# edouardoyallon/acco

Hardware: NVIDIA H100
Metric: tokens/sec (device-timed, max over ranks) Llama ACCO bf16 sharded-Adam, 8x1024 tokens per GPU per micro-batch (higher is better)
Workload: dtype bf16

## Files before the change

### acco_b200/csrc/attention_wgmma.cu

```cuda
#include <cuda.h>
#include <cuda_bf16.h>
#include <cuda_runtime.h>
#include <math.h>
#include <stdint.h>

#include "wgmma.cuh"

namespace acco_attn {

using namespace acco_tc;

constexpr int HD = 64;
constexpr int LDS = HD + 8;
constexpr float LOG2E = 1.4426950408889634f;
constexpr float LN2 = 0.6931471805599453f;

typedef __nv_bfloat16 bf16;

__device__ __forceinline__ uint32_t pack2(float a, float b) {
    __nv_bfloat162 h = __floats2bfloat162_rn(a, b);
    return *reinterpret_cast<uint32_t*>(&h);
}
__device__ __forceinline__ uint32_t ld32(const bf16* p) { return *reinterpret_cast<const uint32_t*>(p); }

__device__ __forceinline__ void mma16816(float (&c)[4], const uint32_t (&a)[4], uint32_t b0, uint32_t b1) {
    asm volatile("mma.sync.aligned.m16n8k16.row.col.f32.bf16.bf16.f32 {%0,%1,%2,%3}, {%4,%5,%6,%7}, {%8,%9}, {%0,%1,%2,%3};"
                 : "+f"(c[0]), "+f"(c[1]), "+f"(c[2]), "+f"(c[3])
                 : "r"(a[0]), "r"(a[1]), "r"(a[2]), "r"(a[3]), "r"(b0), "r"(b1));
}

template <int NB, int KB>
__device__ __forceinline__ void warp_mma_ss(float (&acc)[NB][4], const bf16* A, const bf16* B, int lane) {
    const int g = lane >> 2, t = lane & 3;
#pragma unroll
    for (int kb = 0; kb < KB; ++kb) {
        uint32_t a[4];
        const bf16* a0 = A + g * LDS + kb * 16 + 2 * t;
        a[0] = ld32(a0); a[1] = ld32(a0 + 8 * LDS); a[2] = ld32(a0 + 8); a[3] = ld32(a0 + 8 * LDS + 8);
#pragma unroll
        for (int nb = 0; nb < NB; ++nb) {
            const bf16* b = B + (nb * 8 + g) * LDS + kb * 16 + 2 * t;
            mma16816(acc[nb], a, ld32(b), ld32(b + 8));
        }
    }
}
template <int NB>
__device__ __forceinline__ void warp_mma_rs(float (&acc)[NB][4], const float (&p)[8][4], const bf16* B, int lane) {
    const int g = lane >> 2, t = lane & 3;
#pragma unroll
    for (int kb = 0; kb < 4; ++kb) {
        uint32_t a[4];
        a[0] = pack2(p[2 * kb][0], p[2 * kb][1]);
        a[1] = pack2(p[2 * kb][2], p[2 * kb][3]);
        a[2] = pack2(p[2 * kb + 1][0], p[2 * kb + 1][1]);
        a[3] = pack2(p[2 * kb + 1][2], p[2 * kb + 1][3]);
#pragma unroll
        for (int nb = 0; nb < NB; ++nb) {
            const bf16* b = B + (nb * 8 + g) * LDS + kb * 16 + 2 * t;
            mma16816(acc[nb], a, ld32(b), ld32(b + 8));
        }
    }
}

__device__ __forceinline__ void load_tile(bf16* dst, const bf16* src, long long ld, int rows, int valid, int tid, int nthr) {
    for (int i = tid; i < rows * 8; i += nthr) {
        const int r = i >> 3, c = (i & 7) * 8;
        uint4 v = make_uint4(0, 0, 0, 0);
        if (r < valid) v = *reinterpret_cast<const uint4*>(src + (long long)r * ld + c);
        *reinterpret_cast<uint4*>(dst + r * LDS + c) = v;
    }
}
__device__ __forceinline__ void load_tile_t(bf16* dst, const bf16* src, long long ld, int rows, int tid, int nthr) {
    for (int i = tid; i < rows * 8; i += nthr) {
        const int r = i >> 3, c = (i & 7) * 8;
        const uint4 v = *reinterpret_cast<const uint4*>(src + (long long)r * ld + c);
        const bf16* e = reinterpret_cast<const bf16*>(&v);
#pragma unroll
        for (int j = 0; j < 8; ++j) dst[(c + j) * LDS + r] = e[j];
    }
}

__device__ __forceinline__ bool visible(int q, int kv, int window) { return kv <= q && kv > q - window; }

struct FwdParams {
    CUtensorMap map_q;
    CUtensorMap map_k;
    CUtensorMap map_v;
    bf16* o;
    long long ld_o;
    float* lse;
    int B, S, Hq, Hk, window;
    float scale;
    const int* seg;
};

constexpr int FWD_Q = 128, FWD_KV = 64, FWD_THREADS = 256;
constexpr int FWD_TILE_KV = FWD_KV * HD * 2;
constexpr int FWD_SMEM = FWD_Q * HD * 2 + 2 * 2 * FWD_TILE_KV + 1024  + 64 ;

__device__ __forceinline__ void wgmma_m64n64k16_rs_tb(float (&d)[32], const uint32_t (&a)[4], uint64_t db) {
    asm volatile(
        "{\n\t.reg .pred p;\n\tsetp.ne.b32 p, %37, 0;\n\twgmma.mma_async.sync.aligned.m64n64k16.f32.bf16.bf16 "
// ... 116 lines not shown
                a[3] = pack2(sc[8 * kk + 6], sc[8 * kk + 7]);
                wgmma_m64n64k16_rs_tb(o, a, make_smem_desc(v_addr + kk * 2048, 8192 >> 4, 1024 >> 4));
            }
            wgmma_commit();
            wgmma_wait<0>();
            reg_fence(o);
        }
        __syncthreads();
        if (tid == 0 && j + 2 <= j_hi) issue(j + 2);
    }
#pragma unroll
    for (int r = 0; r < 2; ++r) {
        const int q = qr[r];
        const float inv = l_run[r] > 0.f ? 1.f / l_run[r] : 0.f;
        bf16* dst = P.o + ((long long)row0 + q) * P.ld_o + h * HD + 2 * t;
#pragma unroll
        for (int nb = 0; nb < 8; ++nb)
            *reinterpret_cast<uint32_t*>(dst + nb * 8) = pack2(o[4 * nb + 2 * r] * inv, o[4 * nb + 2 * r + 1] * inv);
        if (t == 0) P.lse[((long long)b * P.Hq + h) * P.S + q] = (m_run[r] + log2f(l_run[r])) * LN2;
    }
}

struct BwdParams {
    const bf16 *q, *k, *v;
    long long ld;
    const bf16* d_o;
    long long ld_do;
    const float *lse, *delta;
    float* dq;
    bf16 *dk, *dv;
    int B, S, Hq, Hk, window;
    float scale;
    const int* seg;
};

constexpr int BWD_KV = 64, BWD_Q = 64, BWD_THREADS = 128;
constexpr int BWD_SMEM = 8 * 64 * LDS * 2 + 2 * BWD_Q * 4;
constexpr int BWD_SMEM_SEG = BWD_SMEM + (BWD_Q + 1) * 4;

template <bool kSeg>
__global__ void __launch_bounds__(BWD_THREADS) attn_bwd_kernel(const BwdParams P) {
    extern __shared__ __align__(16) uint8_t smem_raw[];
    bf16* sK = reinterpret_cast<bf16*>(smem_raw);
    bf16* sKt = sK + 64 * LDS;
    bf16* sV = sKt + 64 * LDS;
    bf16* sQ = sV + 64 * LDS;
    bf16* sQt = sQ + 64 * LDS;
    bf16* sdO = sQt + 64 * LDS;
    bf16* sdOt = sdO + 64 * LDS;
    bf16* sdS = sdOt + 64 * LDS;
    float* sL = reinterpret_cast<float*>(sdS + 64 * LDS);
    float* sD = sL + BWD_Q;
    int* sSeg = reinterpret_cast<int*>(sD + BWD_Q);
    const int nb_k = blockIdx.x, hk = blockIdx.y, b = blockIdx.z;
    const int G = P.Hq / P.Hk;
    const int tid = threadIdx.x, warp = tid >> 5, lane = tid & 31, g = lane >> 2, t = lane & 3;
    const int kv0 = nb_k * BWD_KV;
    const long long row0 = (long long)b * P.S;
    load_tile(sK, P.k + (row0 + kv0) * P.ld + hk * HD, P.ld, BWD_KV, BWD_KV, tid, BWD_THREADS);
    load_tile_t(sKt, P.k + (row0 + kv0) * P.ld + hk * HD, P.ld, BWD_KV, tid, BWD_THREADS);
    load_tile(sV, P.v + (row0 + kv0) * P.ld + hk * HD, P.ld, BWD_KV, BWD_KV, tid, BWD_THREADS);
    const float c = P.scale * LOG2E;
    float dk[8][4], dv[8][4];
#pragma unroll
    for (int i = 0; i < 8; ++i)
#pragma unroll
        for (int e = 0; e < 4; ++e) dk[i][e] = dv[i][e] = 0.f;
    const int kr[2] = {kv0 + warp * 16 + g, kv0 + warp * 16 + g + 8};
    const int m_lo = kv0 / BWD_Q;
    const int m_hi = min(P.S / BWD_Q - 1, (kv0 + BWD_KV - 1 + P.window - 1) / BWD_Q);
    for (int gi = 0; gi < G; ++gi) {
        const int hq = hk * G + gi;
        for (int m = m_lo; m <= m_hi; ++m) {
            const int q0 = m * BWD_Q;
            __syncthreads();
            load_tile(sQ, P.q + (row0 + q0) * P.ld + hq * HD, P.ld, BWD_Q, BWD_Q, tid, BWD_THREADS);
            load_tile_t(sQt, P.q + (row0 + q0) * P.ld + hq * HD, P.ld, BWD_Q, tid, BWD_THREADS);
            load_tile(sdO, P.d_o + (row0 + q0) * P.ld_do + hq * HD, P.ld_do, BWD_Q, BWD_Q, tid, BWD_THREADS);
            load_tile_t(sdOt, P.d_o + (row0 + q0) * P.ld_do + hq * HD, P.ld_do, BWD_Q, tid, BWD_THREADS);
            if (tid < BWD_Q) {
                const long long li = ((long long)b * P.Hq + hq) * P.S + q0 + tid;
                sL[tid] = P.lse[li] * LOG2E;
                sD[tid] = P.delta[li];
                if constexpr (kSeg) sSeg[tid] = P.seg[row0 + q0 + tid];
            }
            if (kSeg && tid == BWD_Q) sSeg[BWD_Q] = m == m_hi || P.seg[row0 + q0 + BWD_Q] > kv0 + BWD_KV - 1;
            __syncthreads();
            float s[8][4], dp[8][4];
#pragma unroll
            for (int i = 0; i < 8; ++i)
#pragma unroll
                for (int e = 0; e < 4; ++e) s[i][e] = dp[i][e] = 0.f;
            warp_mma_ss<8, 4>(s, sK + warp * 16 * LDS, sQ, lane);
            warp_mma_ss<8, 4>(dp, sV + warp * 16 * LDS, sdO, lane);
#pragma unroll
            for (int nb = 0; nb < 8; ++nb)
#pragma unroll
                for (int e = 0; e < 4; ++e) {
                    const int ql = nb * 8 + 2 * t + (e & 1), q = q0 + ql, r = e >> 1;
                    const float p = visible(q, kr[r], P.window) && (!kSeg || kr[r] >= sSeg[ql]) ? exp2f(s[nb][e] * c - sL[ql]) : 0.f;
                    const float pb = __bfloat162float(__float2bfloat16(p));
                    s[nb][e] = pb;
                    dp[nb][e] = __bfloat162float(__float2bfloat16(p * (dp[nb][e] - sD[ql]) * P.scale));
                }
#pragma unroll
            for (int nb = 0; nb < 8; ++nb)
#pragma unroll
                for (int e = 0; e < 4; ++e) {
                    const int ql = nb * 8 + 2 * t + (e & 1), kl = warp * 16 + g + 8 * (e >> 1);
                    sdS[ql * LDS + kl] = __float2bfloat16(dp[nb][e]);
                }
            warp_mma_rs<8>(dv, s, sdOt, lane);
            warp_mma_rs<8>(dk, dp, sQt, lane);
            __syncthreads();
            float dq[8][4];
#pragma unroll
            for (int i = 0; i < 8; ++i) dq[i][0] = dq[i][1] = dq[i][2] = dq[i][3] = 0.f;
            warp_mma_ss<8, 4>(dq, sdS + warp * 16 * LDS, sKt, lane);
#pragma unroll
            for (int r = 0; r < 2; ++r) {
                float* dst = P.dq + (row0 + q0 + warp * 16 + g + 8 * r) * (long long)(P.Hq * HD) + hq * HD + 2 * t;
#pragma unroll
                for (int nb = 0; nb < 8; ++nb) {
                    atomicAdd(dst + nb * 8, dq[nb][2 * r]);
                    atomicAdd(dst + nb * 8 + 1, dq[nb][2 * r + 1]);
                }
            }
            if (kSeg && sSeg[BWD_Q]) break;
        }
    }
#pragma unroll
    for (int r = 0; r < 2; ++r) {
        const long long off = (row0 + kr[r]) * (long long)(P.Hk * HD) + hk * HD + 2 * t;
#pragma unroll
        for (int nb = 0; nb < 8; ++nb) {
            *reinterpret_cast<uint32_t*>(P.dk + off + nb * 8) = pack2(dk[nb][2 * r], dk[nb][2 * r + 1]);
            *reinterpret_cast<uint32_t*>(P.dv + off + nb * 8) = pack2(dv[nb][2 * r], dv[nb][2 * r + 1]);
        }
    }
}

__global__ void __launch_bounds__(256) attn_delta_kernel(const bf16* __restrict__ o, const bf16* __restrict__ d_o, long long ld_o,
                                                         long long ld_do, float* __restrict__ delta, int B, int S, int Hq) {
    const long long item = ((long long)blockIdx.x * blockDim.x + threadIdx.x) >> 3;
    const int part = threadIdx.x & 7;
    const long long n_items = (long long)B * S * Hq;
    float acc = 0.f;
    long long row = 0;
    int h = 0;
    if (item < n_items) {
        row = item / Hq;
        h = (int)(item - row * Hq);
        const uint4 a = *reinterpret_cast<const uint4*>(o + row * ld_o + h * HD + part * 8);
        const uint4 d = *reinterpret_cast<const uint4*>(d_o + row * ld_do + h * HD + part * 8);
        const __nv_bfloat162* a2 = reinterpret_cast<const __nv_bfloat162*>(&a);
        const __nv_bfloat162* d2 = reinterpret_cast<const __nv_bfloat162*>(&d);
#pragma unroll
        for (int i = 0; i < 4; ++i) {
            const float2 x = __bfloat1622float2(a2[i]), y = __bfloat1622float2(d2[i]);
            acc += x.x * y.x + x.y * y.y;
// ... 27 lines not shown
    static int fwd_attr = (int)cudaFuncSetAttribute(attn_fwd_kernel<false>, cudaFuncAttributeMaxDynamicSharedMemorySize, FWD_SMEM);
    static int fwd_attr_seg = (int)cudaFuncSetAttribute(attn_fwd_kernel<true>, cudaFuncAttributeMaxDynamicSharedMemorySize, FWD_SMEM);
    if (fwd_attr) return fwd_attr;
    if (fwd_attr_seg) return fwd_attr_seg;
    FwdParams P;
    const uint64_t rows = (uint64_t)B * S;
    int rc = acco_gemm::make_map_typed(&P.map_q, q, (uint64_t)Hq * HD, rows, (uint64_t)ld, HD, FWD_Q, 2);
    if (!rc) rc = acco_gemm::make_map_typed(&P.map_k, k, (uint64_t)Hk * HD, rows, (uint64_t)ld, HD, FWD_KV, 2);
    if (!rc) rc = acco_gemm::make_map_typed(&P.map_v, v, (uint64_t)Hk * HD, rows, (uint64_t)ld, HD, FWD_KV, 2);
    if (rc) return rc;
    P.o = (bf16*)o; P.ld_o = ld_o; P.lse = lse;
    P.B = B; P.S = S; P.Hq = Hq; P.Hk = Hk; P.window = eff_window(S, window); P.scale = scale; P.seg = seg;
    if (seg)
        attn_fwd_kernel<true><<<dim3(S / FWD_Q, Hq, B), FWD_THREADS, FWD_SMEM, st>>>(P);
    else
        attn_fwd_kernel<false><<<dim3(S / FWD_Q, Hq, B), FWD_THREADS, FWD_SMEM, st>>>(P);
    return (int)cudaGetLastError();
}

extern "C" int acco_attn_bwd(const void* q, const void* k, const void* v, long long ld, const void* o, long long ld_o, const void* d_o,
                             long long ld_do, const float* lse, float* delta, float* dq_acc, void* dk, void* dv, int B, int S, int Hq, int Hk, int D,
                             float scale, int window, const int* seg, cudaStream_t st) {
    using namespace acco_attn;
    if (!shape_ok(B, S, Hq, Hk, D, scale) || !aligned(q, ld) || !aligned(k, ld) || !aligned(v, ld) || !aligned(o, ld_o) || !aligned(d_o, ld_do))
        return -1;
    static int attr_rc = (int)cudaFuncSetAttribute(attn_bwd_kernel<false>, cudaFuncAttributeMaxDynamicSharedMemorySize, BWD_SMEM);
    static int attr_rc_seg = (int)cudaFuncSetAttribute(attn_bwd_kernel<true>, cudaFuncAttributeMaxDynamicSharedMemorySize, BWD_SMEM_SEG);
    if (attr_rc) return attr_rc;
    if (attr_rc_seg) return attr_rc_seg;
    const long long items = (long long)B * S * Hq;
    attn_delta_kernel<<<(unsigned)((items * 8 + 255) / 256), 256, 0, st>>>((const bf16*)o, (const bf16*)d_o, ld_o, ld_do, delta, B, S, Hq);
    if (cudaMemsetAsync(dq_acc, 0, (size_t)items * HD * sizeof(float), st) != cudaSuccess) return -6;
    BwdParams P{(const bf16*)q, (const bf16*)k, (const bf16*)v, ld, (const bf16*)d_o, ld_do, lse, delta, dq_acc, (bf16*)dk, (bf16*)dv,
                B, S, Hq, Hk, eff_window(S, window), scale, seg};
    if (seg)
        attn_bwd_kernel<true><<<dim3(S / BWD_KV, Hk, B), BWD_THREADS, BWD_SMEM_SEG, st>>>(P);
    else
        attn_bwd_kernel<false><<<dim3(S / BWD_KV, Hk, B), BWD_THREADS, BWD_SMEM, st>>>(P);
    return (int)cudaGetLastError();
}
```

### acco_b200/csrc/bindings.cpp

```cpp
#include <torch/extension.h>
#include <ATen/cuda/CUDAContext.h>
#include <c10/cuda/CUDAGuard.h>
#include <cuda_runtime.h>

#include <cmath>
#include <cstdlib>
#include <vector>

extern "C" {
int acco_norm_grid(int T, int H, int sms, int backward);
int acco_rmsnorm_fwd(const void* a, const void* r, const void* w, void* y, void* h, float* rstd, int T, int H, float eps,
                     int grid, cudaStream_t st);
int acco_rmsnorm_bwd(const void* dy, const void* dh_extra, const void* h, const void* w, const float* rstd, void* dh,
                     float* dw_partial, float* dw_out, void* dw_accum_bf16, int T, int H, int grid, cudaStream_t st);
int acco_rope_pack_bwd(const void* dq, const void* dk, const void* dv, const long long* strides, void* dqkv, const float* cos_t,
                       const float* sin_t, int B, int S, int Hq, int Hk, int D, int sms, cudaStream_t st);
int acco_rope_qkv(void* qkv, const float* cos_t, const float* sin_t, int T, int S, int n_rot, int n_total, int D, int inverse,
                  int sms, cudaStream_t st);
int acco_swiglu_fwd(const void* gu, void* out, long long T, int I, int sms, cudaStream_t st);
int acco_swiglu_bwd(const void* dout, const void* gu, void* dgu, long long T, int I, int sms, cudaStream_t st);
int acco_ce_fwd(const void* logits, const long long* labels, float* lse, float* row_loss, float* loss, float* inv_n, long long T,
                int V, int Vp, long long ignore_index, cudaStream_t st);
int acco_ce_bwd(void* logits, const long long* labels, const float* lse, const float* scale, long long T, int V, int Vp,
                long long ignore_index, cudaStream_t st);
int acco_layernorm_grid(int T, int H, int sms, int backward);
int acco_layernorm_fwd(const void* a, const void* r, const void* w, const void* b, void* y, void* h, float* mean, float* rstd, int T, int H,
                       float eps, int grid, cudaStream_t st);
int acco_layernorm_bwd(const void* dy, const void* dh_extra, const void* h, const void* w, const float* mean, const float* rstd, void* dh,
                       float* partial, float* dwdb_out, void* dw_accum_bf16, void* db_accum_bf16, int T, int H, int grid, cudaStream_t st);
int acco_gelu_fwd(const void* x, void* y, long long n, int sms, cudaStream_t st);
int acco_gelu_bwd(const void* dy, const void* x, void* dx, long long n, int sms, cudaStream_t st);
int acco_debug_occupy(unsigned long long ns, int ctas, float* sink, cudaStream_t st);
int acco_round_params_size();
int acco_gemm_run(const void* a, long long lda, int a_mn, const void* b, long long ldb, int b_mn, void* d, long long ldd, const void* bias,
                  int M, int N, int K, int accumulate, int bn_req, int splits_req, int pm_req, int pn_req, int msub_req, int sms, cudaStream_t st);
int acco_gemm_tn_gather(const void* x, const void* w_local, void* y, int M, int N, int K, const void* const* peers, int n_peers,
                        const int* tile_owner, uint32_t* flags, uint32_t* epoch, uint32_t* done, int sms, cudaStream_t st);
long long acco_gemm_map_encodes();
int acco_gemm_max_clusters(int cl, int sms);
// ... 163 lines not shown
    TORCH_CHECK(acco_gelu_fwd(x.data_ptr(), y.data_ptr(), x.numel(), sm_count(), stream()) == 0, "gelu: numel must be a multiple of 8");
    return y;
}
torch::Tensor gelu_bwd(torch::Tensor dy, torch::Tensor x) {
    check_bf16(x, "x"); check_bf16(dy, "dy");
    const c10::cuda::CUDAGuard guard(x.device());
    auto dx = torch::empty_like(x);
    TORCH_CHECK(acco_gelu_bwd(dy.data_ptr(), x.data_ptr(), dx.data_ptr(), x.numel(), sm_count(), stream()) == 0, "gelu: numel must be a multiple of 8");
    return dx;
}

void rope_qkv_inplace(torch::Tensor qkv, torch::Tensor cos_t, torch::Tensor sin_t, int64_t B, int64_t S, int64_t n_rot,
                      int64_t n_total, int64_t D, bool inverse) {
    check_bf16(qkv, "qkv"); check_f32(cos_t, "cos"); check_f32(sin_t, "sin");
    const c10::cuda::CUDAGuard guard(qkv.device());
    TORCH_CHECK(qkv.numel() == B * S * n_total * D, "qkv has the wrong number of elements");
    TORCH_CHECK(cos_t.size(0) >= S && cos_t.size(1) == D / 2, "cos/sin tables must be [>=S, D/2]");
    TORCH_CHECK(acco_rope_qkv(qkv.data_ptr(), cos_t.data_ptr<float>(), sin_t.data_ptr<float>(), (int)(B * S), (int)S, (int)n_rot,
                              (int)n_total, (int)D, inverse ? 1 : 0, sm_count(), stream()) == 0,
                "rope: head_dim must be a multiple of 16");
}

torch::Tensor rope_pack_bwd(torch::Tensor dq, torch::Tensor dk, torch::Tensor dv, torch::Tensor cos_t, torch::Tensor sin_t) {
    TORCH_CHECK(dq.is_cuda() && dq.scalar_type() == torch::kBFloat16 && dk.scalar_type() == torch::kBFloat16 && dv.scalar_type() == torch::kBFloat16, "bf16 CUDA grads expected");
    TORCH_CHECK(dq.stride(3) == 1 && dk.stride(3) == 1 && dv.stride(3) == 1, "head dim must be contiguous");
    check_f32(cos_t, "cos"); check_f32(sin_t, "sin");
    const c10::cuda::CUDAGuard guard(dq.device());
    const int64_t B = dq.size(0), S = dq.size(1), Hq = dq.size(2), D = dq.size(3), Hk = dk.size(2);
    for (auto* t : {&dq, &dk, &dv}) TORCH_CHECK((t->stride(0) % 8 == 0) && (t->stride(1) % 8 == 0) && (t->stride(2) % 8 == 0) && ((uintptr_t)t->data_ptr() % 16 == 0), "16-byte aligned strides required");
    auto out = torch::empty({B * S, (Hq + 2 * Hk) * D}, dq.options());
    long long st[9] = {dq.stride(0), dq.stride(1), dq.stride(2), dk.stride(0), dk.stride(1), dk.stride(2), dv.stride(0), dv.stride(1), dv.stride(2)};
    TORCH_CHECK(acco_rope_pack_bwd(dq.data_ptr(), dk.data_ptr(), dv.data_ptr(), st, out.data_ptr(), cos_t.data_ptr<float>(), sin_t.data_ptr<float>(),
                                   (int)B, (int)S, (int)Hq, (int)Hk, (int)D, sm_count(), stream()) == 0, "rope_pack_bwd: head_dim must be a multiple of 16");
    return out;
}

torch::Tensor swiglu_fwd(torch::Tensor gu) {
    check_bf16(gu, "gate_up");
    const c10::cuda::CUDAGuard guard(gu.device());
    const int64_t T = gu.size(0), I = gu.size(1) / 2;
    auto out = torch::empty({T, I}, gu.options());
    TORCH_CHECK(acco_swiglu_fwd(gu.data_ptr(), out.data_ptr(), T, (int)I, sm_count(), stream()) == 0, "swiglu: I must be a multiple of 8");
    return out;
}

torch::Tensor swiglu_bwd(torch::Tensor dout, torch::Tensor gu) {
    check_bf16(dout, "dout"); check_bf16(gu, "gate_up");
    const c10::cuda::CUDAGuard guard(gu.device());
    const int64_t T = gu.size(0), I = gu.size(1) / 2;
    auto dgu = torch::empty_like(gu);
    TORCH_CHECK(acco_swiglu_bwd(dout.data_ptr(), gu.data_ptr(), dgu.data_ptr(), T, (int)I, sm_count(), stream()) == 0, "swiglu: I must be a multiple of 8");
    return dgu;
}

std::vector<torch::Tensor> ce_fwd(torch::Tensor logits, torch::Tensor labels, int64_t V, int64_t ignore_index) {
    check_bf16(logits, "logits");
// ... 323 lines not shown
```

### acco_b200/csrc/elementwise.cu

```cuda
#include <stdlib.h>

#include "common.cuh"

namespace acco {

ACCO_DEVINL void load_cs(const float* __restrict__ cos_t, const float* __restrict__ sin_t, int pos, int half, int v, float (&c)[8],
                         float (&s)[8]) {
    const float4* cp = reinterpret_cast<const float4*>(cos_t + (size_t)pos * half + 8 * v);
    const float4* sp = reinterpret_cast<const float4*>(sin_t + (size_t)pos * half + 8 * v);
    const float4 c0 = __ldg(cp), c1 = __ldg(cp + 1), s0 = __ldg(sp), s1 = __ldg(sp + 1);
    c[0] = c0.x; c[1] = c0.y; c[2] = c0.z; c[3] = c0.w; c[4] = c1.x; c[5] = c1.y; c[6] = c1.z; c[7] = c1.w;
    s[0] = s0.x; s[1] = s0.y; s[2] = s0.z; s[3] = s0.w; s[4] = s1.x; s[5] = s1.y; s[6] = s1.z; s[7] = s1.w;
}

__global__ void __launch_bounds__(256) rope_qkv_kernel(__nv_bfloat16* __restrict__ qkv, const float* __restrict__ cos_t,
                                                       const float* __restrict__ sin_t, int T, int S, int n_rot,
                                                       int n_total, int D, float sign) {
    const int half = D >> 1;
    const int vph = half >> 3;
    const int lane = threadIdx.x & 31;
    const int v = lane % vph, hg = lane / vph, hstep = 32 / vph;
    const int warps = (gridDim.x * blockDim.x) >> 5;
    for (int t = (blockIdx.x * blockDim.x + threadIdx.x) >> 5; t < T; t += warps) {
        float c[8], s[8];
        load_cs(cos_t, sin_t, t % S, half, v, c, s);
        __nv_bfloat16* row = qkv + (size_t)t * n_total * D + 8 * v;
        for (int h = hg; h < n_rot; h += hstep) {
            __nv_bfloat16* p1 = row + (size_t)h * D;
            float x1[8], x2[8], o1[8], o2[8];
            unpack8(ld_vec(p1), x1);
            unpack8(ld_vec(p1 + half), x2);
#pragma unroll
            for (int j = 0; j < 8; ++j) {
                const float sj = sign * s[j];
                o1[j] = x1[j] * c[j] - x2[j] * sj;
                o2[j] = x2[j] * c[j] + x1[j] * sj;
            }
            st_vec(p1, pack8(o1));
            st_vec(p1 + half, pack8(o2));
        }
    }
}

struct PackSrc {
    const __nv_bfloat16* ptr[3];
    long long sb[3], ss[3], sh[3];
};
__global__ void __launch_bounds__(256) rope_pack_bwd_kernel(PackSrc src, __nv_bfloat16* __restrict__ dqkv,
                                                            const float* __restrict__ cos_t, const float* __restrict__ sin_t,
                                                            int B, int S, int Hq, int Hk, int D) {
    const int half = D >> 1;
    const int vph = half >> 3;
    const int n_total = Hq + 2 * Hk;
    const int lane = threadIdx.x & 31;
    const int v = lane % vph, hg = lane / vph, hstep = 32 / vph;
    const int warps = (gridDim.x * blockDim.x) >> 5;
    const int T = B * S;
    for (int t = (blockIdx.x * blockDim.x + threadIdx.x) >> 5; t < T; t += warps) {
        const int s = t % S, b = t / S;
        float c[8], sn[8];
        load_cs(cos_t, sin_t, s, half, v, c, sn);
        __nv_bfloat16* orow = dqkv + (size_t)t * n_total * D + 8 * v;
        for (int head = hg; head < n_total; head += hstep) {
            int which, h;
            if (head < Hq) { which = 0; h = head; }
            else if (head < Hq + Hk) { which = 1; h = head - Hq; }
            else { which = 2; h = head - Hq - Hk; }
            const __nv_bfloat16* p1 = src.ptr[which] + b * src.sb[which] + s * src.ss[which] + h * src.sh[which] + 8 * v;
            float x1[8], x2[8];
            unpack8(ld_stream(p1), x1);
            unpack8(ld_stream(p1 + half), x2);
            __nv_bfloat16* o1 = orow + (size_t)head * D;
            if (which == 2) {
                st_vec(o1, pack8(x1));
                st_vec(o1 + half, pack8(x2));
            } else {
                float r1[8], r2[8];
#pragma unroll
                for (int j = 0; j < 8; ++j) {
                    r1[j] = x1[j] * c[j] + x2[j] * sn[j];
                    r2[j] = x2[j] * c[j] - x1[j] * sn[j];
                }
                st_vec(o1, pack8(r1));
                st_vec(o1 + half, pack8(r2));
            }
        }
    }
}

__global__ void __launch_bounds__(256) swiglu_fwd_kernel(const __nv_bfloat16* __restrict__ gu, __nv_bfloat16* __restrict__ out,
                                                         long long T, int I) {
    const int vpr = I >> 3;
    const long long total = T * vpr;
    for (long long idx = (long long)blockIdx.x * blockDim.x + threadIdx.x; idx < total;
// ... 39 lines not shown
        st_stream(o + I, pack8(du));
    }
}

static int grid_for(long long work_items, int threads, int sms) {
    long long want = (work_items + threads - 1) / threads;
    long long cap = (long long)sms * (2048 / threads) * 4;
    if (want < 1) want = 1;
    return (int)(want < cap ? want : cap);
}

}

extern "C" int acco_rope_qkv(void* qkv, const float* cos_t, const float* sin_t, int T, int S, int n_rot, int n_total, int D,
                             int inverse, int sms, cudaStream_t st) {
    if (D % 16 != 0 || (32 % (D / 16)) != 0) return -1;
    const long long work = (long long)T * 32;
    acco::rope_qkv_kernel<<<acco::grid_for(work, 256, sms), 256, 0, st>>>((__nv_bfloat16*)qkv, cos_t, sin_t, T, S, n_rot,
                                                                          n_total, D, inverse ? -1.f : 1.f);
    return 0;
}

extern "C" int acco_rope_pack_bwd(const void* dq, const void* dk, const void* dv, const long long* strides ,
                                  void* dqkv, const float* cos_t, const float* sin_t, int B, int S, int Hq, int Hk, int D, int sms,
                                  cudaStream_t st) {
    if (D % 16 != 0 || (32 % (D / 16)) != 0) return -1;
    acco::PackSrc src;
    src.ptr[0] = (const __nv_bfloat16*)dq; src.ptr[1] = (const __nv_bfloat16*)dk; src.ptr[2] = (const __nv_bfloat16*)dv;
    for (int i = 0; i < 3; ++i) { src.sb[i] = strides[3 * i]; src.ss[i] = strides[3 * i + 1]; src.sh[i] = strides[3 * i + 2]; }
    const long long work = (long long)B * S * 32;
    acco::rope_pack_bwd_kernel<<<acco::grid_for(work, 256, sms), 256, 0, st>>>(src, (__nv_bfloat16*)dqkv, cos_t, sin_t, B, S, Hq, Hk, D);
    return 0;
}

extern "C" int acco_swiglu_fwd(const void* gu, void* out, long long T, int I, int sms, cudaStream_t st) {
    if (I % 8 != 0) return -1;
    acco::swiglu_fwd_kernel<<<acco::grid_for(T * (I / 8), 256, sms), 256, 0, st>>>((const __nv_bfloat16*)gu,
                                                                                    (__nv_bfloat16*)out, T, I);
    return 0;
}

extern "C" int acco_swiglu_bwd(const void* dout, const void* gu, void* dgu, long long T, int I, int sms, cudaStream_t st) {
    if (I % 8 != 0) return -1;
    acco::swiglu_bwd_kernel<<<acco::grid_for(T * (I / 8), 256, sms), 256, 0, st>>>(
        (const __nv_bfloat16*)dout, (const __nv_bfloat16*)gu, (__nv_bfloat16*)dgu, T, I);
    return 0;
}

namespace acco {
__global__ void __launch_bounds__(256, 4) occupy_kernel(unsigned long long ns, float* sink) {
    float v[56];
#pragma unroll
    for (int i = 0; i < 56; ++i) v[i] = (float)(threadIdx.x + i);
    unsigned long long t0, t;
// ... 25 lines not shown
```

### acco_b200/ops/attention.py

```python
from __future__ import annotations

import logging
import math
import os
from typing import Optional, Tuple

import torch
import torch.nn.functional as F

_SDPA_BACKENDS = None


def _sdpa_ctx():
    global _SDPA_BACKENDS
    from torch.nn.attention import SDPBackend, sdpa_kernel
    if _SDPA_BACKENDS is None:
        _SDPA_BACKENDS = [SDPBackend.CUDNN_ATTENTION, SDPBackend.FLASH_ATTENTION, SDPBackend.EFFICIENT_ATTENTION, SDPBackend.MATH]
    try:
        return sdpa_kernel(_SDPA_BACKENDS, set_priority=True)
    except TypeError:
        return sdpa_kernel(_SDPA_BACKENDS)


def _window_mask(S: int, window: int, device) -> torch.Tensor:
# ... 266 lines not shown
            _log_seg_fallback(B, S, Hq, Hk, D)
        ctx.own = None
        x = qkv.detach().view(B, S, Hq + 2 * Hk, D)
        with torch.enable_grad():
            q = x[:, :, :Hq].transpose(1, 2).requires_grad_()
            k = x[:, :, Hq:Hq + Hk].transpose(1, 2).requires_grad_()
            v = x[:, :, Hq + Hk:].transpose(1, 2).requires_grad_()
            out = _attend(q, k, v, scale, window, Hk != Hq, seg)
        ctx.inner = (out, q, k, v)
        return out.detach().transpose(1, 2).reshape(B * S, Hq * D)

    @staticmethod
    def backward(ctx, dout):
        from . import count_launch, load_ext
        C = load_ext(required=True)
        cos, sin = ctx.saved_tensors
        B, S, Hq, Hk, D, rb, rs = ctx.dims
        if ctx.own is not None:
            qkv, o, lse, sc, window, seg = ctx.own
            ctx.own = None
            extra = () if seg is None else (seg,)
            dq, dk, dv = C.attn_bwd(qkv, o, dout.contiguous(), lse, B, S, Hq, Hk, D, sc, window, *extra)
            count_launch("attn_bwd" if seg is None else "attn_bwd_seg", 2)
            dqkv = C.rope_pack_bwd(dq.to(torch.bfloat16).view(rb, rs, Hq, D), dk.view(rb, rs, Hk, D), dv.view(rb, rs, Hk, D), cos, sin)
            count_launch("rope_pack_bwd")
            return (dqkv,) + (None,) * 11
        out, q, k, v = ctx.inner
        ctx.inner = None
        do = dout.reshape(B, S, Hq, D).transpose(1, 2)
        dq, dk, dv = torch.autograd.grad(out, (q, k, v), do)
        dq, dk, dv = (t if t.stride(-1) == 1 else t.contiguous() for t in (dq, dk, dv))
        dq, dk, dv = (t.transpose(1, 2) for t in (dq, dk, dv))
        if rb != B:
            dq, dk, dv = (t.reshape(rb, rs, t.shape[2], D) for t in (dq, dk, dv))
        dqkv = C.rope_pack_bwd(dq, dk, dv, cos, sin)
        count_launch("rope_pack_bwd")
        return (dqkv,) + (None,) * 11


def rope_causal_attention(qkv: torch.Tensor, cos: torch.Tensor, sin: torch.Tensor, B: int, S: int, Hq: int, Hk: int, D: int,
                          seg: Optional[torch.Tensor] = None) -> torch.Tensor:
    from . import use_kernels
    from .rope import rope_qkv_ref
    if use_kernels(qkv):
        if seg is not None or (torch.is_grad_enabled() and qkv.requires_grad):
            return _RopeAttentionFn.apply(qkv, cos, sin, B, S, Hq, Hk, D, True, None, None, seg)
        from . import count_launch, load_ext
# ... 23 lines not shown
```

Before: 317,500.

## Rewrite attention backward with TMA producer warp and wgmma, fuse fp32 dq into rope pack

The attention backward kernel moves from mma.sync with manual shared-memory tile and transpose loads to a warpgroup wgmma design. A dedicated producer thread issues TMA loads of Q, dO, lse, delta and seg into a two-stage mbarrier pipeline. dq is accumulated with vectorized red.global.add.v4, and segment-masked blocks are bounded by a binary search instead of an early break. rope_pack_bwd now reads fp32 dq directly, removing the separate bf16 cast kernel, at the cost of more complex swizzled layouts and synchronisation.

```diff
diff --git a/acco_b200/csrc/attention_wgmma.cu b/acco_b200/csrc/attention_wgmma.cu
--- a/acco_b200/csrc/attention_wgmma.cu
+++ b/acco_b200/csrc/attention_wgmma.cu
@@ -11,7 +11,6 @@
 using namespace acco_tc;
 
 constexpr int HD = 64;
-constexpr int LDS = HD + 8;
 constexpr float LOG2E = 1.4426950408889634f;
 constexpr float LN2 = 0.6931471805599453f;
 
@@ -20,64 +19,6 @@
 __device__ __forceinline__ uint32_t pack2(float a, float b) {
     __nv_bfloat162 h = __floats2bfloat162_rn(a, b);
     return *reinterpret_cast<uint32_t*>(&h);
-}
-__device__ __forceinline__ uint32_t ld32(const bf16* p) { return *reinterpret_cast<const uint32_t*>(p); }
-
-__device__ __forceinline__ void mma16816(float (&c)[4], const uint32_t (&a)[4], uint32_t b0, uint32_t b1) {
-    asm volatile("mma.sync.aligned.m16n8k16.row.col.f32.bf16.bf16.f32 {%0,%1,%2,%3}, {%4,%5,%6,%7}, {%8,%9}, {%0,%1,%2,%3};"
-                 : "+f"(c[0]), "+f"(c[1]), "+f"(c[2]), "+f"(c[3])
-                 : "r"(a[0]), "r"(a[1]), "r"(a[2]), "r"(a[3]), "r"(b0), "r"(b1));
-}
-
-template <int NB, int KB>
-__device__ __forceinline__ void warp_mma_ss(float (&acc)[NB][4], const bf16* A, const bf16* B, int lane) {
-    const int g = lane >> 2, t = lane & 3;
-#pragma unroll
-    for (int kb = 0; kb < KB; ++kb) {
-        uint32_t a[4];
-        const bf16* a0 = A + g * LDS + kb * 16 + 2 * t;
-        a[0] = ld32(a0); a[1] = ld32(a0 + 8 * LDS); a[2] = ld32(a0 + 8); a[3] = ld32(a0 + 8 * LDS + 8);
-#pragma unroll
-        for (int nb = 0; nb < NB; ++nb) {
-            const bf16* b = B + (nb * 8 + g) * LDS + kb * 16 + 2 * t;
-            mma16816(acc[nb], a, ld32(b), ld32(b + 8));
-        }
-    }
-}
-template <int NB>
-__device__ __forceinline__ void warp_mma_rs(float (&acc)[NB][4], const float (&p)[8][4], const bf16* B, int lane) {
-    const int g = lane >> 2, t = lane & 3;
-#pragma unroll
-    for (int kb = 0; kb < 4; ++kb) {
-        uint32_t a[4];
-        a[0] = pack2(p[2 * kb][0], p[2 * kb][1]);
-        a[1] = pack2(p[2 * kb][2], p[2 * kb][3]);
-        a[2] = pack2(p[2 * kb + 1][0], p[2 * kb + 1][1]);
-        a[3] = pack2(p[2 * kb + 1][2], p[2 * kb + 1][3]);
-#pragma unroll
-        for (int nb = 0; nb < NB; ++nb) {
-            const bf16* b = B + (nb * 8 + g) * LDS + kb * 16 + 2 * t;
-            mma16816(acc[nb], a, ld32(b), ld32(b + 8));
-        }
-    }
-}
-
-__device__ __forceinline__ void load_tile(bf16* dst, const bf16* src, long long ld, int rows, int valid, int tid, int nthr) {
-    for (int i = tid; i < rows * 8; i += nthr) {
-        const int r = i >> 3, c = (i & 7) * 8;
-        uint4 v = make_uint4(0, 0, 0, 0);
-        if (r < valid) v = *reinterpret_cast<const uint4*>(src + (long long)r * ld + c);
-        *reinterpret_cast<uint4*>(dst + r * LDS + c) = v;
-    }
-}
-__device__ __forceinline__ void load_tile_t(bf16* dst, const bf16* src, long long ld, int rows, int tid, int nthr) {
-    for (int i = tid; i < rows * 8; i += nthr) {
-        const int r = i >> 3, c = (i & 7) * 8;
-        const uint4 v = *reinterpret_cast<const uint4*>(src + (long long)r * ld + c);
-        const bf16* e = reinterpret_cast<const bf16*>(&v);
-#pragma unroll
-        for (int j = 0; j < 8; ++j) dst[(c + j) * LDS + r] = e[j];
-    }
 }
 
 __device__ __forceinline__ bool visible(int q, int kv, int window) { return kv <= q && kv > q - window; }
@@ -240,10 +181,10 @@
 }
 
 struct BwdParams {
-    const bf16 *q, *k, *v;
-    long long ld;
-    const bf16* d_o;
-    long long ld_do;
+    CUtensorMap map_q;
+    CUtensorMap map_k;
+    CUtensorMap map_v;
+    CUtensorMap map_do;
     const float *lse, *delta;
     float* dq;
     bf16 *dk, *dv;
@@ -252,99 +193,171 @@
     const int* seg;
 };
 
-constexpr int BWD_KV = 64, BWD_Q = 64, BWD_THREADS = 128;
-constexpr int BWD_SMEM = 8 * 64 * LDS * 2 + 2 * BWD_Q * 4;
-constexpr int BWD_SMEM_SEG = BWD_SMEM + (BWD_Q + 1) * 4;
+constexpr int BWD_KV = 64, BWD_Q = 64, BWD_STAGES = 2;
+constexpr int BWD_THREADS = 160;
+constexpr int BWD_TILE = 64 * HD * 2;
+constexpr int BWD_STAGE = 2 * BWD_TILE + 3 * BWD_Q * 4;
+constexpr int BWD_SMEM = 3 * BWD_TILE + BWD_STAGES * BWD_STAGE + 1024  + 64 ;
+
+__device__ __forceinline__ void bulk_load(void* dst, const void* src, uint32_t bytes, uint64_t* bar) {
+    asm volatile("cp.async.bulk.shared::cluster.global.mbarrier::complete_tx::bytes [%0], [%1], %2, [%3];" ::"r"(smem_u32(dst)), "l"(src),
+                 "r"(bytes), "r"(smem_u32(bar))
+                 : "memory");
+}
+__device__ __forceinline__ void red_add_v4(float* p, float a, float b, float c, float d) {
+    asm volatile("red.global.add.v4.f32 [%0], {%1, %2, %3, %4};" ::"l"(p), "f"(a), "f"(b), "f"(c), "f"(d) : "memory");
+}
 
 template <bool kSeg>
-__global__ void __launch_bounds__(BWD_THREADS) attn_bwd_kernel(const BwdParams P) {
-    extern __shared__ __align__(16) uint8_t smem_raw[];
-    bf16* sK = reinterpret_cast<bf16*>(smem_raw);
-    bf16* sKt = sK + 64 * LDS;
-    bf16* sV = sKt + 64 * LDS;
-    bf16* sQ = sV + 64 * LDS;
-    bf16* sQt = sQ + 64 * LDS;
-    bf16* sdO = sQt + 64 * LDS;
-    bf16* sdOt = sdO + 64 * LDS;
-    bf16* sdS = sdOt + 64 * LDS;
-    float* sL = reinterpret_cast<float*>(sdS + 64 * LDS);
-    float* sD = sL + BWD_Q;
-    int* sSeg = reinterpret_cast<int*>(sD + BWD_Q);
+__device__ __forceinline__ int bwd_last_block(const BwdParams& P, long long row0, int kv0) {
+    const int m_hi = min(P.S / BWD_Q - 1, (kv0 + BWD_KV - 1 + P.window - 1) / BWD_Q);
+    if constexpr (!kSeg) return m_hi;
+    int lo = kv0 / BWD_Q, hi = m_hi;
+    while (lo < hi) {
+        const int mid = (lo + hi + 1) >> 1;
+        if (P.seg[row0 + mid * BWD_Q] <= kv0 + BWD_KV - 1) lo = mid;
+        else hi = mid - 1;
+    }
+    return lo;
+}
+
+template <bool kSeg>
+__global__ void __launch_bounds__(BWD_THREADS) attn_bwd_kernel(const __grid_constant__ BwdParams P) {
+    extern __shared__ uint8_t smem_raw[];
+    uint8_t* smem = (uint8_t*)(((uintptr_t)smem_raw + 1023) & ~(uintptr_t)1023);
+    uint8_t* sK = smem;
+    uint8_t* sV = sK + BWD_TILE;
+    uint8_t* sdS = sV + BWD_TILE;
+    uint8_t* sStage = sdS + BWD_TILE;
+    uint64_t* full = (uint64_t*)(sStage + BWD_STAGES * BWD_STAGE);
+    uint64_t* empty = full + BWD_STAGES;
+    uint64_t* kv_full = empty + BWD_STAGES;
     const int nb_k = blockIdx.x, hk = blockIdx.y, b = blockIdx.z;
     const int G = P.Hq / P.Hk;
-    const int tid = threadIdx.x, warp = tid >> 5, lane = tid & 31, g = lane >> 2, t = lane & 3;
+    const int tid = threadIdx.x;
     const int kv0 = nb_k * BWD_KV;
     const long long row0 = (long long)b * P.S;
-    load_tile(sK, P.k + (row0 + kv0) * P.ld + hk * HD, P.ld, BWD_KV, BWD_KV, tid, BWD_THREADS);
-    load_tile_t(sKt, P.k + (row0 + kv0) * P.ld + hk * HD, P.ld, BWD_KV, tid, BWD_THREADS);
-    load_tile(sV, P.v + (row0 + kv0) * P.ld + hk * HD, P.ld, BWD_KV, BWD_KV, tid, BWD_THREADS);
+    const int m_lo = kv0 / BWD_Q, m_end = bwd_last_block<kSeg>(P, row0, kv0);
+    if (tid == 0) {
+        for (int s = 0; s < BWD_STAGES; ++s) {
+            mbar_init(&full[s], 1);
+            mbar_init(&empty[s], 128);
+        }
+        mbar_init(kv_full, 1);
+        asm volatile("fence.mbarrier_init.release.cluster;" ::: "memory");
+    }
+    __syncthreads();
+    if (tid >= 128) {
+        if (tid != 128) return;
+        mbar_expect_tx(kv_full, 2 * BWD_TILE);
+        tma_load_2d(&P.map_k, kv_full, sK, hk * HD, (int)row0 + kv0);
+        tma_load_2d(&P.map_v, kv_full, sV, hk * HD, (int)row0 + kv0);
+        constexpr uint32_t bytes = 2 * BWD_TILE + (kSeg ? 3 : 2) * BWD_Q * 4;
+        int it = 0;
+        for (int gi = 0; gi < G; ++gi) {
+            const int hq = hk * G + gi;
+            for (int m = m_lo; m <= m_end; ++m, ++it) {
+                const int s = it % BWD_STAGES, q0 = m * BWD_Q;
+                if (it >= BWD_STAGES) mbar_wait(&empty[s], (uint32_t)((it / BWD_STAGES - 1) & 1));
+                uint8_t* st = sStage + s * BWD_STAGE;
+                mbar_expect_tx(&full[s], bytes);
+                tma_load_2d(&P.map_q, &full[s], st, hq * HD, (int)row0 + q0);
+                tma_load_2d(&P.map_do, &full[s], st + BWD_TILE, hq * HD, (int)row0 + q0);
+                const long long li = ((long long)b * P.Hq + hq) * P.S + q0;
+                bulk_load(st + 2 * BWD_TILE, P.lse + li, BWD_Q * 4, &full[s]);
+                bulk_load(st + 2 * BWD_TILE + BWD_Q * 4, P.delta + li, BWD_Q * 4, &full[s]);
+                if constexpr (kSeg) bulk_load(st + 2 * BWD_TILE + 2 * BWD_Q * 4, P.seg + row0 + q0, BWD_Q * 4, &full[s]);
+            }
+        }
+        return;
+    }
+    const int warp = tid >> 5, lane = tid & 31, g = lane >> 2, t = lane & 3;
     const float c = P.scale * LOG2E;
-    float dk[8][4], dv[8][4];
-#pragma unroll
-    for (int i = 0; i < 8; ++i)
-#pragma unroll
-        for (int e = 0; e < 4; ++e) dk[i][e] = dv[i][e] = 0.f;
+    float dk[32], dv[32];
+#pragma unroll
+    for (int i = 0; i < 32; ++i) dk[i] = dv[i] = 0.f;
     const int kr[2] = {kv0 + warp * 16 + g, kv0 + warp * 16 + g + 8};
-    const int m_lo = kv0 / BWD_Q;
-    const int m_hi = min(P.S / BWD_Q - 1, (kv0 + BWD_KV - 1 + P.window - 1) / BWD_Q);
+    const uint32_t k_addr = smem_u32(sK), v_addr = smem_u32(sV), ds_addr = smem_u32(sdS);
+    mbar_wait(kv_full, 0);
+    int it = 0;
     for (int gi = 0; gi < G; ++gi) {
         const int hq = hk * G + gi;
-        for (int m = m_lo; m <= m_hi; ++m) {
-            const int q0 = m * BWD_Q;
-            __syncthreads();
-            load_tile(sQ, P.q + (row0 + q0) * P.ld + hq * HD, P.ld, BWD_Q, BWD_Q, tid, BWD_THREADS);
-            load_tile_t(sQt, P.q + (row0 + q0) * P.ld + hq * HD, P.ld, BWD_Q, tid, BWD_THREADS);
-            load_tile(sdO, P.d_o + (row0 + q0) * P.ld_do + hq * HD, P.ld_do, BWD_Q, BWD_Q, tid, BWD_THREADS);
-            load_tile_t(sdOt, P.d_o + (row0 + q0) * P.ld_do + hq * HD, P.ld_do, BWD_Q, tid, BWD_THREADS);
-            if (tid < BWD_Q) {
-                const long long li = ((long long)b * P.Hq + hq) * P.S + q0 + tid;
-                sL[tid] = P.lse[li] * LOG2E;
-                sD[tid] = P.delta[li];
-                if constexpr (kSeg) sSeg[tid] = P.seg[row0 + q0 + tid];
-            }
-            if (kSeg && tid == BWD_Q) sSeg[BWD_Q] = m == m_hi || P.seg[row0 + q0 + BWD_Q] > kv0 + BWD_KV - 1;
-            __syncthreads();
-            float s[8][4], dp[8][4];
-#pragma unroll
-            for (int i = 0; i < 8; ++i)
-#pragma unroll
-                for (int e = 0; e < 4; ++e) s[i][e] = dp[i][e] = 0.f;
-            warp_mma_ss<8, 4>(s, sK + warp * 16 * LDS, sQ, lane);
-            warp_mma_ss<8, 4>(dp, sV + warp * 16 * LDS, sdO, lane);
-#pragma unroll
-            for (int nb = 0; nb < 8; ++nb)
-#pragma unroll
-                for (int e = 0; e < 4; ++e) {
-                    const int ql = nb * 8 + 2 * t + (e & 1), q = q0 + ql, r = e >> 1;
-                    const float p = visible(q, kr[r], P.window) && (!kSeg || kr[r] >= sSeg[ql]) ? exp2f(s[nb][e] * c - sL[ql]) : 0.f;
-                    const float pb = __bfloat162float(__float2bfloat16(p));
-                    s[nb][e] = pb;
-                    dp[nb][e] = __bfloat162float(__float2bfloat16(p * (dp[nb][e] - sD[ql]) * P.scale));
+        for (int m = m_lo; m <= m_end; ++m, ++it) {
+            const int s = it % BWD_STAGES, q0 = m * BWD_Q;
+            const uint8_t* st = sStage + s * BWD_STAGE;
+            const uint32_t q_addr = smem_u32(st), do_addr = q_addr + BWD_TILE;
+            const float* sL = reinterpret_cast<const float*>(st + 2 * BWD_TILE);
+            const float* sD = sL + BWD_Q;
+            const int* sSeg = reinterpret_cast<const int*>(sD + BWD_Q);
+            mbar_wait(&full[s], (uint32_t)((it / BWD_STAGES) & 1));
+            float sc[32], dp[32];
+#pragma unroll
+            for (int i = 0; i < 32; ++i) sc[i] = dp[i] = 0.f;
+            wgmma_fence();
+#pragma unroll
+            for (int k = 0; k < HD / 16; ++k)
+                wgmma_m64n64k16<0, 0>(sc, make_smem_desc(k_addr + k * 32, 1, 1024 >> 4), make_smem_desc(q_addr + k * 32, 1, 1024 >> 4), 1u);
+            wgmma_commit();
+#pragma unroll
+            for (int k = 0; k < HD / 16; ++k)
+                wgmma_m64n64k16<0, 0>(dp, make_smem_desc(v_addr + k * 32, 1, 1024 >> 4), make_smem_desc(do_addr + k * 32, 1, 1024 >> 4), 1u);
+            wgmma_commit();
+            wgmma_wait<0>();
+            reg_fence(sc);
+            reg_fence(dp);
+            uint32_t pa[16], da[16];
+#pragma unroll
+            for (int i = 0; i < 16; ++i) {
+                const int ql = (i >> 1) * 8 + 2 * t, r = i & 1;
+                float p[2], ds[2];
+#pragma unroll
+                for (int e = 0; e < 2; ++e) {
+                    p[e] = visible(q0 + ql + e, kr[r], P.window) && (!kSeg || kr[r] >= sSeg[ql + e]) ? exp2f(sc[2 * i + e] * c - sL[ql + e] * LOG2E)
+                                                                                                     : 0.f;
+                    ds[e] = p[e] * (dp[2 * i + e] - sD[ql + e]) * P.scale;
                 }
-#pragma unroll
-            for (int nb = 0; nb < 8; ++nb)
-#pragma unroll
-                for (int e = 0; e < 4; ++e) {
-                    const int ql = nb * 8 + 2 * t + (e & 1), kl = warp * 16 + g + 8 * (e >> 1);
-                    sdS[ql * LDS + kl] = __float2bfloat16(dp[nb][e]);
-                }
-            warp_mma_rs<8>(dv, s, sdOt, lane);
-            warp_mma_rs<8>(dk, dp, sQt, lane);
-            __syncthreads();
-            float dq[8][4];
-#pragma unroll
-            for (int i = 0; i < 8; ++i) dq[i][0] = dq[i][1] = dq[i][2] = dq[i][3] = 0.f;
-            warp_mma_ss<8, 4>(dq, sdS + warp * 16 * LDS, sKt, lane);
-#pragma unroll
-            for (int r = 0; r < 2; ++r) {
-                float* dst = P.dq + (row0 + q0 + warp * 16 + g + 8 * r) * (long long)(P.Hq * HD) + hq * HD + 2 * t;
-#pragma unroll
-                for (int nb = 0; nb < 8; ++nb) {
-                    atomicAdd(dst + nb * 8, dq[nb][2 * r]);
-                    atomicAdd(dst + nb * 8 + 1, dq[nb][2 * r + 1]);
-                }
-            }
-            if (kSeg && sSeg[BWD_Q]) break;
+                pa[i] = pack2(p[0], p[1]);
+                da[i] = pack2(ds[0], ds[1]);
+            }
+#pragma unroll
+            for (int i = 0; i < 16; ++i) {
+                const int kl = warp * 16 + g + 8 * (i & 1), nb = i >> 1;
+                st_shared_u32(ds_addr + kl * 128 + ((nb ^ (kl & 7)) << 4) + 4 * t, da[i]);
+            }
+            fence_async_smem();
+            wgmma_fence();
+#pragma unroll
+            for (int kk = 0; kk < BWD_Q / 16; ++kk) {
+                const uint32_t a[4] = {pa[4 * kk], pa[4 * kk + 1], pa[4 * kk + 2], pa[4 * kk + 3]};
+                wgmma_m64n64k16_rs_tb(dv, a, make_smem_desc(do_addr + kk * 2048, 8192 >> 4, 1024 >> 4));
+            }
+#pragma unroll
+            for (int kk = 0; kk < BWD_Q / 16; ++kk) {
+                const uint32_t a[4] = {da[4 * kk], da[4 * kk + 1], da[4 * kk + 2], da[4 * kk + 3]};
+                wgmma_m64n64k16_rs_tb(dk, a, make_smem_desc(q_addr + kk * 2048, 8192 >> 4, 1024 >> 4));
+            }
+            wgmma_commit();
+            named_barrier(1, 128);
+            float dq[32];
+            wgmma_fence();
+#pragma unroll
+            for (int kk = 0; kk < BWD_KV / 16; ++kk)
+                wgmma_m64n64k16<1, 1>(dq, make_smem_desc(ds_addr + kk * 2048, 8192 >> 4, 1024 >> 4),
+                                      make_smem_desc(k_addr + kk * 2048, 8192 >> 4, 1024 >> 4), kk > 0 ? 1u : 0u);
+            wgmma_commit();
+            wgmma_wait<0>();
+            reg_fence(dq);
+            reg_fence(dk);
+            reg_fence(dv);
+            mbar_arrive(&empty[s]);
+            const bool odd = t & 1;
+            float* dst = P.dq + (row0 + q0 + warp * 16 + g + (odd ? 8 : 0)) * (long long)(P.Hq * HD) + hq * HD + 2 * (t & ~1);
+#pragma unroll
+            for (int nb = 0; nb < 8; ++nb) {
+                const float s0 = odd ? dq[4 * nb] : dq[4 * nb + 2], s1 = odd ? dq[4 * nb + 1] : dq[4 * nb + 3];
+                const float r0 = __shfl_xor_sync(0xffffffffu, s0, 1), r1 = __shfl_xor_sync(0xffffffffu, s1, 1);
+                red_add_v4(dst + nb * 8, odd ? r0 : dq[4 * nb], odd ? r1 : dq[4 * nb + 1], odd ? dq[4 * nb + 2] : r0, odd ? dq[4 * nb + 3] : r1);
+            }
         }
     }
 #pragma unroll
@@ -352,8 +365,8 @@
         const long long off = (row0 + kr[r]) * (long long)(P.Hk * HD) + hk * HD + 2 * t;
 #pragma unroll
         for (int nb = 0; nb < 8; ++nb) {
-            *reinterpret_cast<uint32_t*>(P.dk + off + nb * 8) = pack2(dk[nb][2 * r], dk[nb][2 * r + 1]);
-            *reinterpret_cast<uint32_t*>(P.dv + off + nb * 8) = pack2(dv[nb][2 * r], dv[nb][2 * r + 1]);
+            *reinterpret_cast<uint32_t*>(P.dk + off + nb * 8) = pack2(dk[4 * nb + 2 * r], dk[4 * nb + 2 * r + 1]);
+            *reinterpret_cast<uint32_t*>(P.dv + off + nb * 8) = pack2(dv[4 * nb + 2 * r], dv[4 * nb + 2 * r + 1]);
         }
     }
 }
@@ -427,19 +440,27 @@
                              long long ld_do, const float* lse, float* delta, float* dq_acc, void* dk, void* dv, int B, int S, int Hq, int Hk, int D,
                              float scale, int window, const int* seg, cudaStream_t st) {
     using namespace acco_attn;
-    if (!shape_ok(B, S, Hq, Hk, D, scale) || !aligned(q, ld) || !aligned(k, ld) || !aligned(v, ld) || !aligned(o, ld_o) || !aligned(d_o, ld_do))
+    if (!shape_ok(B, S, Hq, Hk, D, scale) || !aligned(q, ld) || !aligned(k, ld) || !aligned(v, ld) || !aligned(o, ld_o) || !aligned(d_o, ld_do) ||
+        !aligned(lse, 0) || !aligned(delta, 0) || !aligned(dq_acc, 0) || (seg && !aligned(seg, 0)))
         return -1;
     static int attr_rc = (int)cudaFuncSetAttribute(attn_bwd_kernel<false>, cudaFuncAttributeMaxDynamicSharedMemorySize, BWD_SMEM);
-    static int attr_rc_seg = (int)cudaFuncSetAttribute(attn_bwd_kernel<true>, cudaFuncAttributeMaxDynamicSharedMemorySize, BWD_SMEM_SEG);
+    static int attr_rc_seg = (int)cudaFuncSetAttribute(attn_bwd_kernel<true>, cudaFuncAttributeMaxDynamicSharedMemorySize, BWD_SMEM);
     if (attr_rc) return attr_rc;
     if (attr_rc_seg) return attr_rc_seg;
     const long long items = (long long)B * S * Hq;
+    BwdParams P;
+    const uint64_t rows = (uint64_t)B * S;
+    int rc = acco_gemm::make_map_typed(&P.map_q, q, (uint64_t)Hq * HD, rows, (uint64_t)ld, HD, BWD_Q, 2);
+    if (!rc) rc = acco_gemm::make_map_typed(&P.map_k, k, (uint64_t)Hk * HD, rows, (uint64_t)ld, HD, BWD_KV, 2);
+    if (!rc) rc = acco_gemm::make_map_typed(&P.map_v, v, (uint64_t)Hk * HD, rows, (uint64_t)ld, HD, BWD_KV, 2);
+    if (!rc) rc = acco_gemm::make_map_typed(&P.map_do, d_o, (uint64_t)Hq * HD, rows, (uint64_t)ld_do, HD, BWD_Q, 2);
+    if (rc) return rc;
+    P.lse = lse; P.delta = delta; P.dq = dq_acc; P.dk = (bf16*)dk; P.dv = (bf16*)dv;
+    P.B = B; P.S = S; P.Hq = Hq; P.Hk = Hk; P.window = eff_window(S, window); P.scale = scale; P.seg = seg;
     attn_delta_kernel<<<(unsigned)((items * 8 + 255) / 256), 256, 0, st>>>((const bf16*)o, (const bf16*)d_o, ld_o, ld_do, delta, B, S, Hq);
     if (cudaMemsetAsync(dq_acc, 0, (size_t)items * HD * sizeof(float), st) != cudaSuccess) return -6;
-    BwdParams P{(const bf16*)q, (const bf16*)k, (const bf16*)v, ld, (const bf16*)d_o, ld_do, lse, delta, dq_acc, (bf16*)dk, (bf16*)dv,
-                B, S, Hq, Hk, eff_window(S, window), scale, seg};
     if (seg)
-        attn_bwd_kernel<true><<<dim3(S / BWD_KV, Hk, B), BWD_THREADS, BWD_SMEM_SEG, st>>>(P);
+        attn_bwd_kernel<true><<<dim3(S / BWD_KV, Hk, B), BWD_THREADS, BWD_SMEM, st>>>(P);
     else
         attn_bwd_kernel<false><<<dim3(S / BWD_KV, Hk, B), BWD_THREADS, BWD_SMEM, st>>>(P);
     return (int)cudaGetLastError();
diff --git a/acco_b200/csrc/bindings.cpp b/acco_b200/csrc/bindings.cpp
--- a/acco_b200/csrc/bindings.cpp
+++ b/acco_b200/csrc/bindings.cpp
@@ -14,7 +14,7 @@
 int acco_rmsnorm_bwd(const void* dy, const void* dh_extra, const void* h, const void* w, const float* rstd, void* dh,
                      float* dw_partial, float* dw_out, void* dw_accum_bf16, int T, int H, int grid, cudaStream_t st);
 int acco_rope_pack_bwd(const void* dq, const void* dk, const void* dv, const long long* strides, void* dqkv, const float* cos_t,
-                       const float* sin_t, int B, int S, int Hq, int Hk, int D, int sms, cudaStream_t st);
+                       const float* sin_t, int B, int S, int Hq, int Hk, int D, int dq_f32, int sms, cudaStream_t st);
 int acco_rope_qkv(void* qkv, const float* cos_t, const float* sin_t, int T, int S, int n_rot, int n_total, int D, int inverse,
                   int sms, cudaStream_t st);
 int acco_swiglu_fwd(const void* gu, void* out, long long T, int I, int sms, cudaStream_t st);
@@ -224,16 +224,19 @@
 }
 
 torch::Tensor rope_pack_bwd(torch::Tensor dq, torch::Tensor dk, torch::Tensor dv, torch::Tensor cos_t, torch::Tensor sin_t) {
-    TORCH_CHECK(dq.is_cuda() && dq.scalar_type() == torch::kBFloat16 && dk.scalar_type() == torch::kBFloat16 && dv.scalar_type() == torch::kBFloat16, "bf16 CUDA grads expected");
+    const bool dq_f32 = dq.scalar_type() == torch::kFloat32;
+    TORCH_CHECK(dq.is_cuda() && (dq_f32 || dq.scalar_type() == torch::kBFloat16) && dk.scalar_type() == torch::kBFloat16 &&
+                dv.scalar_type() == torch::kBFloat16, "bf16 CUDA grads expected (dq may be fp32)");
     TORCH_CHECK(dq.stride(3) == 1 && dk.stride(3) == 1 && dv.stride(3) == 1, "head dim must be contiguous");
     check_f32(cos_t, "cos"); check_f32(sin_t, "sin");
     const c10::cuda::CUDAGuard guard(dq.device());
     const int64_t B = dq.size(0), S = dq.size(1), Hq = dq.size(2), D = dq.size(3), Hk = dk.size(2);
     for (auto* t : {&dq, &dk, &dv}) TORCH_CHECK((t->stride(0) % 8 == 0) && (t->stride(1) % 8 == 0) && (t->stride(2) % 8 == 0) && ((uintptr_t)t->data_ptr() % 16 == 0), "16-byte aligned strides required");
-    auto out = torch::empty({B * S, (Hq + 2 * Hk) * D}, dq.options());
+    auto out = torch::empty({B * S, (Hq + 2 * Hk) * D}, dk.options());
     long long st[9] = {dq.stride(0), dq.stride(1), dq.stride(2), dk.stride(0), dk.stride(1), dk.stride(2), dv.stride(0), dv.stride(1), dv.stride(2)};
     TORCH_CHECK(acco_rope_pack_bwd(dq.data_ptr(), dk.data_ptr(), dv.data_ptr(), st, out.data_ptr(), cos_t.data_ptr<float>(), sin_t.data_ptr<float>(),
-                                   (int)B, (int)S, (int)Hq, (int)Hk, (int)D, sm_count(), stream()) == 0, "rope_pack_bwd: head_dim must be a multiple of 16");
+                                   (int)B, (int)S, (int)Hq, (int)Hk, (int)D, dq_f32 ? 1 : 0, sm_count(), stream()) == 0,
+                "rope_pack_bwd: head_dim must be a multiple of 16");
     return out;
 }
 
diff --git a/acco_b200/csrc/elementwise.cu b/acco_b200/csrc/elementwise.cu
--- a/acco_b200/csrc/elementwise.cu
+++ b/acco_b200/csrc/elementwise.cu
@@ -43,9 +43,23 @@
 }
 
 struct PackSrc {
-    const __nv_bfloat16* ptr[3];
+    const void* ptr[3];
     long long sb[3], ss[3], sh[3];
 };
+template <bool kQF32>
+ACCO_DEVINL void load_grad(const PackSrc& src, int which, long long off, int half, float (&x1)[8], float (&x2)[8]) {
+    if (kQF32 && which == 0) {
+        const float* p = reinterpret_cast<const float*>(src.ptr[0]) + off;
+        const float4 a = ld_f4_stream(p), b = ld_f4_stream(p + 4), c = ld_f4_stream(p + half), d = ld_f4_stream(p + half + 4);
+        x1[0] = a.x; x1[1] = a.y; x1[2] = a.z; x1[3] = a.w; x1[4] = b.x; x1[5] = b.y; x1[6] = b.z; x1[7] = b.w;
+        x2[0] = c.x; x2[1] = c.y; x2[2] = c.z; x2[3] = c.w; x2[4] = d.x; x2[5] = d.y; x2[6] = d.z; x2[7] = d.w;
+    } else {
+        const __nv_bfloat16* p = reinterpret_cast<const __nv_bfloat16*>(src.ptr[which]) + off;
+        unpack8(ld_stream(p), x1);
+        unpack8(ld_stream(p + half), x2);
+    }
+}
+template <bool kQF32>
 __global__ void __launch_bounds__(256) rope_pack_bwd_kernel(PackSrc src, __nv_bfloat16* __restrict__ dqkv,
                                                             const float* __restrict__ cos_t, const float* __restrict__ sin_t,
                                                             int B, int S, int Hq, int Hk, int D) {
@@ -66,10 +80,8 @@
             if (head < Hq) { which = 0; h = head; }
             else if (head < Hq + Hk) { which = 1; h = head - Hq; }
             else { which = 2; h = head - Hq - Hk; }
-            const __nv_bfloat16* p1 = src.ptr[which] + b * src.sb[which] + s * src.ss[which] + h * src.sh[which] + 8 * v;
             float x1[8], x2[8];
-            unpack8(ld_stream(p1), x1);
-            unpack8(ld_stream(p1 + half), x2);
+            load_grad<kQF32>(src, which, b * src.sb[which] + s * src.ss[which] + h * src.sh[which] + 8 * v, half, x1, x2);
             __nv_bfloat16* o1 = orow + (size_t)head * D;
             if (which == 2) {
                 st_vec(o1, pack8(x1));
@@ -155,14 +167,17 @@
 }
 
 extern "C" int acco_rope_pack_bwd(const void* dq, const void* dk, const void* dv, const long long* strides ,
-                                  void* dqkv, const float* cos_t, const float* sin_t, int B, int S, int Hq, int Hk, int D, int sms,
+                                  void* dqkv, const float* cos_t, const float* sin_t, int B, int S, int Hq, int Hk, int D, int dq_f32, int sms,
                                   cudaStream_t st) {
     if (D % 16 != 0 || (32 % (D / 16)) != 0) return -1;
     acco::PackSrc src;
-    src.ptr[0] = (const __nv_bfloat16*)dq; src.ptr[1] = (const __nv_bfloat16*)dk; src.ptr[2] = (const __nv_bfloat16*)dv;
+    src.ptr[0] = dq; src.ptr[1] = dk; src.ptr[2] = dv;
     for (int i = 0; i < 3; ++i) { src.sb[i] = strides[3 * i]; src.ss[i] = strides[3 * i + 1]; src.sh[i] = strides[3 * i + 2]; }
     const long long work = (long long)B * S * 32;
-    acco::rope_pack_bwd_kernel<<<acco::grid_for(work, 256, sms), 256, 0, st>>>(src, (__nv_bfloat16*)dqkv, cos_t, sin_t, B, S, Hq, Hk, D);
+    if (dq_f32)
+        acco::rope_pack_bwd_kernel<true><<<acco::grid_for(work, 256, sms), 256, 0, st>>>(src, (__nv_bfloat16*)dqkv, cos_t, sin_t, B, S, Hq, Hk, D);
+    else
+        acco::rope_pack_bwd_kernel<false><<<acco::grid_for(work, 256, sms), 256, 0, st>>>(src, (__nv_bfloat16*)dqkv, cos_t, sin_t, B, S, Hq, Hk, D);
     return 0;
 }
 
diff --git a/acco_b200/ops/attention.py b/acco_b200/ops/attention.py
--- a/acco_b200/ops/attention.py
+++ b/acco_b200/ops/attention.py
@@ -312,7 +312,7 @@
             extra = () if seg is None else (seg,)
             dq, dk, dv = C.attn_bwd(qkv, o, dout.contiguous(), lse, B, S, Hq, Hk, D, sc, window, *extra)
             count_launch("attn_bwd" if seg is None else "attn_bwd_seg", 2)
-            dqkv = C.rope_pack_bwd(dq.to(torch.bfloat16).view(rb, rs, Hq, D), dk.view(rb, rs, Hk, D), dv.view(rb, rs, Hk, D), cos, sin)
+            dqkv = C.rope_pack_bwd(dq.view(rb, rs, Hq, D), dk.view(rb, rs, Hk, D), dv.view(rb, rs, Hk, D), cos, sin)
             count_launch("rope_pack_bwd")
             return (dqkv,) + (None,) * 11
         out, q, k, v = ctx.inner
```

Measured after the change: 319,700, median of 6. About the same (+0.7%).
